# vLAR-group/OGC

Measured on AMD Instinct MI355X. Metric: point-clouds/sec (8192 pts) segnet fwd+bwd, higher is better.
Workload: dtype f32; 1 GPU; C4 KITTI-SF train_seg unsup: segnet_kitti fwd + OGC loss (dynamic+smooth+invariance) + bwd + Adam, 4 samples x 4 views x 8192 pts per GPU; n_point=8192, n_slot=10, parallelism=dp1, optimizer_stepped=True

## Files before the change

ogc_amd/csrc/neighbour_loss.hip:

```cpp
#include "ogc_common.h"

namespace {

constexpr int SUBL = 8;

__device__ __forceinline__ float sgn(float x) { return (float)((x > 0.0f) - (x < 0.0f)); }

template <int P>
__global__ __launch_bounds__(256) void nc_fwd_kernel(int n, int c, int k, const float *__restrict__ mask,
                                                     const int *__restrict__ idx, float *__restrict__ out) {
    const int b = blockIdx.y;
    const int sub = threadIdx.x & (SUBL - 1);
    const int i = blockIdx.x * (256 / SUBL) + (threadIdx.x >> 3);
    const float *mb = mask + (size_t)b * n * c;
    float acc = 0.0f;
    if (i < n) {
        const float *mi = mb + (size_t)i * c;
        const int *row = idx + ((size_t)b * n + i) * k;
        for (int j = sub; j < k; j += SUBL) {
            const float *mj = mb + (size_t)row[j] * c;
            float s = 0.0f;
            for (int ch = 0; ch < c; ++ch) {
                const float d = mi[ch] - mj[ch];
                s += P == 1 ? fabsf(d) : d * d;
            }
            acc += P == 1 ? s : sqrtf(s);
        }
    }
#pragma unroll
    for (int off = 1; off < SUBL; off <<= 1) acc += __shfl_xor(acc, off, 64);
    if (i < n && sub == 0) out[(size_t)b * n + i] = acc / (float)k;
}

constexpr unsigned REV_FIRST = 0x80000000u;

__device__ __forceinline__ bool rev_keep(const int *__restrict__ idx, long long e, int n, int k, int &dst, int &src,
                                         bool &first_dup) {
    const int j = (int)(e % k);
    src = (int)((e / k) % n);
    dst = idx[e];
    const int first = idx[e - j];
    first_dup = j > 0 && dst == first;
    return dst != src && !first_dup;
}

template <bool ROWWISE>
__global__ __launch_bounds__(256) void rev_count_kernel(long long total, int n, int k, const int *__restrict__ idx,
                                                        int *__restrict__ deg, int *__restrict__ mult) {
    const long long e = (long long)blockIdx.x * 256 + threadIdx.x;
    const bool in = e < total;
    int dst = 0, src = 0;
    bool dup = false, keep = false;
    long long b = 0;
    if (in) {
        b = e / ((long long)n * k);
        keep = rev_keep(idx, e, n, k, dst, src, dup);
    }
    if (keep) atomicAdd(&deg[b * (n + 1) + dst], 1);
    const bool extra = in && !keep && dup && dst != src;
    if (ROWWISE) {
        const unsigned long long copies = __builtin_amdgcn_ballot_w64(extra);
        const int lane = threadIdx.x & 63, row0 = lane & ~(k - 1);
        if (in && lane == row0) {
            const unsigned long long row_mask = k == 64 ? ~0ull : ((1ull << k) - 1ull) << row0;
            mult[b * n + src] = 1 + __popcll(copies & row_mask);
        }
    } else if (extra) {
        atomicAdd(&mult[b * n + src], 1);
    }
}

__global__ __launch_bounds__(1024) void rev_scan_kernel(int n, int *__restrict__ deg_to_start, int *__restrict__ cursor) {
    __shared__ int part[1024];
    const int t = threadIdx.x, b = blockIdx.x;
    int *d = deg_to_start + (size_t)b * (n + 1);
    int *cur = cursor + (size_t)b * n;
    const int per = (n + 1023) / 1024;
    const int c0 = min(t * per, n), c1 = min(c0 + per, n);
    int sum = 0;
    for (int j = c0; j < c1; ++j) sum += d[j];
    part[t] = sum;
    __syncthreads();
    for (int off = 1; off < 1024; off <<= 1) {
        const int v = t >= off ? part[t - off] : 0;
        __syncthreads();
        part[t] += v;
        __syncthreads();
    }
    int run = t > 0 ? part[t - 1] : 0;
    for (int j = c0; j < c1; ++j) {
        const int cnt = d[j];
        d[j] = run;
        cur[j] = run;
        run += cnt;
    }
    if (t == 1023) d[n] = part[1023];
}

__global__ __launch_bounds__(256) void rev_fill_kernel(long long total, int n, int k, const int *__restrict__ idx,
                                                       int *__restrict__ cursor, int *__restrict__ rev_src) {
    const long long e = (long long)blockIdx.x * 256 + threadIdx.x;
    if (e >= total) return;
    const long long b = e / ((long long)n * k);
    int dst, src;
    bool dup;
    if (!rev_keep(idx, e, n, k, dst, src, dup)) return;
    const int pos = atomicAdd(&cursor[b * n + dst], 1);
    rev_src[b * (long long)n * k + pos] = (int)((unsigned)src | (e % k == 0 ? REV_FIRST : 0u));
}

__global__ __launch_bounds__(256) void rev_sort_kernel(int n, int k, const int *__restrict__ rev_start, int *__restrict__ rev_src) {
    const int j = blockIdx.x * 256 + threadIdx.x, b = blockIdx.y;
    if (j >= n) return;
    const int *rs = rev_start + (size_t)b * (n + 1);
    int *a = rev_src + (size_t)b * n * k;
    const int lo = rs[j], hi = rs[j + 1];
    for (int i = lo + 1; i < hi; ++i) {
        const int v = a[i];
        const unsigned key = (unsigned)v & ~REV_FIRST;
        int q = i - 1;
        while (q >= lo && ((unsigned)a[q] & ~REV_FIRST) > key) {
            a[q + 1] = a[q];
            --q;
        }
        a[q + 1] = v;
    }
}

template <int P>
__device__ __forceinline__ void nc_edge(const float *a, const float *b_, int c, float w, float *g ,
                                        int stride) {
    if (P == 1) {
        for (int ch = 0; ch < c; ++ch) g[ch * stride] += w * sgn(a[ch] - b_[ch]);
    } else {
        float s = 0.0f;
        for (int ch = 0; ch < c; ++ch) { const float d = a[ch] - b_[ch]; s += d * d; }
        const float nrm = sqrtf(s);
        if (nrm > 0.0f) {
            const float inv = w / nrm;
            for (int ch = 0; ch < c; ++ch) g[ch * stride] += inv * (a[ch] - b_[ch]);
        }
    }
}

template <int P>
__global__ __launch_bounds__(256) void nc_bwd_kernel(int n, int c, int k, const float *__restrict__ mask,
                                                     const int *__restrict__ idx, const int *__restrict__ rev_start,
                                                     const int *__restrict__ rev_src,
                                                     const int *__restrict__ rev_mult,
                                                     const float *__restrict__ grad_out,
                                                     float *__restrict__ grad_mask) {
    extern __shared__ float nc_smem[];
    const int b = blockIdx.y;
    const int sub = threadIdx.x & (SUBL - 1);
    const int i = blockIdx.x * (256 / SUBL) + (threadIdx.x >> 3);
    float *g = nc_smem + threadIdx.x;
    for (int ch = 0; ch < c; ++ch) g[ch * 256] = 0.0f;
    const float *mb = mask + (size_t)b * n * c;
    const float *go = grad_out + (size_t)b * n;
    if (i < n) {
        const float *mi = mb + (size_t)i * c;
        const float inv_k = 1.0f / (float)k;
        const int *row = idx + ((size_t)b * n + i) * k;
        const float gi = go[i] * inv_k;
        for (int j = sub; j < k; j += SUBL) nc_edge<P>(mi, mb + (size_t)row[j] * c, c, gi, g, 256);
        const int *rs = rev_start + (size_t)b * (n + 1);
        const int *src = rev_src + (size_t)b * n * k;
        for (int e = rs[i] + sub; e < rs[i + 1]; e += SUBL) {
            const unsigned raw = (unsigned)src[e];
            const int ip = (int)(raw & ~REV_FIRST);
            const float times = (raw & REV_FIRST) ? (float)rev_mult[(size_t)b * n + ip] : 1.0f;
            nc_edge<P>(mb + (size_t)ip * c, mi, c, -go[ip] * inv_k * times, g, 256);
        }
    }
    __syncthreads();
    const int points = 256 / SUBL;
    for (int o = threadIdx.x; o < points * c; o += 256) {
        const int pl = o / c, ch = o % c;
        const int pi = blockIdx.x * points + pl;
        if (pi < n) {
            float s = 0.0f;
#pragma unroll
            for (int l = 0; l < SUBL; ++l) s += nc_smem[ch * 256 + pl * SUBL + l];
            grad_mask[((size_t)b * n + pi) * c + ch] = s;
        }
    }
}

}

extern "C" int ogc_neighbour_consistency_fwd(int b, int n, int c, int k, int p, const float *mask, const int *idx,
                                             float *out, ogc_stream_t stream) {
    OGC_REQUIRE(b >= 0 && n >= 0 && c >= 0 && k >= 0, "ogc_neighbour_consistency_fwd: negative size");
    OGC_REQUIRE(p == 1 || p == 2, "ogc_neighbour_consistency_fwd: norm must be 1 or 2");
    if (b == 0 || n == 0) return OGC_OK;
    OGC_REQUIRE(k > 0, "ogc_neighbour_consistency_fwd: k must be positive");
    OGC_REQUIRE(mask && idx && out, "ogc_neighbour_consistency_fwd: null pointer");
    const dim3 grid(ogc_divup(n, 256 / SUBL), b);
    if (p == 1) hipLaunchKernelGGL(nc_fwd_kernel<1>, grid, dim3(256), 0, (hipStream_t)stream, n, c, k, mask, idx, out);
    else hipLaunchKernelGGL(nc_fwd_kernel<2>, grid, dim3(256), 0, (hipStream_t)stream, n, c, k, mask, idx, out);
    OGC_CHECK_LAUNCH("ogc_neighbour_consistency_fwd");
    return OGC_OK;
}

__global__ __launch_bounds__(256) void fill_ones_kernel(long long total, int *__restrict__ p) {
    const long long e = (long long)blockIdx.x * 256 + threadIdx.x;
    if (e < total) p[e] = 1;
}

extern "C" int ogc_reverse_neighbours(int b, int n, int k, const int *idx, int *rev_start, int *rev_src, int *rev_mult,
                                      int *ws, ogc_stream_t stream) {
    OGC_REQUIRE(b >= 0 && n >= 0 && k >= 0, "ogc_reverse_neighbours: negative size");
    if (b == 0) return OGC_OK;
    OGC_REQUIRE(rev_start, "ogc_reverse_neighbours: null pointer");
    hipStream_t s = (hipStream_t)stream;
    if (ogc_zero_async(rev_start, (size_t)b * (n + 1) * sizeof(int), s) != hipSuccess) {
        ogc_set_error("ogc_reverse_neighbours: zero fill failed");
        return OGC_ERR_LAUNCH;
    }
    const long long total = (long long)b * n * k;
    if (total == 0) return OGC_OK;
    OGC_REQUIRE(idx && rev_src && rev_mult && ws, "ogc_reverse_neighbours: null pointer");
    const unsigned blocks = (unsigned)((total + 255) / 256);
    if (k <= 64 && (k & (k - 1)) == 0) {
        hipLaunchKernelGGL(rev_count_kernel<true>, dim3(blocks), dim3(256), 0, s, total, n, k, idx, rev_start, rev_mult);
    } else {
        hipLaunchKernelGGL(fill_ones_kernel, dim3(ogc_divup(b * n, 256)), dim3(256), 0, s, (long long)b * n, rev_mult);
        hipLaunchKernelGGL(rev_count_kernel<false>, dim3(blocks), dim3(256), 0, s, total, n, k, idx, rev_start,
                           rev_mult);
    }
    hipLaunchKernelGGL(rev_scan_kernel, dim3(b), dim3(1024), 0, s, n, rev_start, ws);
    hipLaunchKernelGGL(rev_fill_kernel, dim3(blocks), dim3(256), 0, s, total, n, k, idx, ws, rev_src);
    if (ogc_deterministic()) hipLaunchKernelGGL(rev_sort_kernel, dim3(ogc_divup(n, 256), b), dim3(256), 0, s, n, k, rev_start, rev_src);
    OGC_CHECK_LAUNCH("ogc_reverse_neighbours");
    return OGC_OK;
}

extern "C" int ogc_neighbour_consistency_bwd(int b, int n, int c, int k, int p, const float *mask, const int *idx,
                                             const int *rev_start, const int *rev_src, const int *rev_mult,
                                             const float *grad_out, float *grad_mask, ogc_stream_t stream) {
    OGC_REQUIRE(b >= 0 && n >= 0 && c >= 0 && k >= 0, "ogc_neighbour_consistency_bwd: negative size");
    OGC_REQUIRE(p == 1 || p == 2, "ogc_neighbour_consistency_bwd: norm must be 1 or 2");
    if (b == 0 || n == 0 || c == 0) return OGC_OK;
    OGC_REQUIRE(k > 0, "ogc_neighbour_consistency_bwd: k must be positive");
    OGC_REQUIRE(c <= 40, "ogc_neighbour_consistency_bwd: more than 40 channels");
    OGC_REQUIRE(mask && idx && rev_start && rev_src && rev_mult && grad_out && grad_mask,
                "ogc_neighbour_consistency_bwd: null pointer");
    const dim3 grid(ogc_divup(n, 256 / SUBL), b);
    const size_t smem = (size_t)c * 256 * sizeof(float);
    if (p == 1)
        hipLaunchKernelGGL(nc_bwd_kernel<1>, grid, dim3(256), smem, (hipStream_t)stream, n, c, k, mask, idx, rev_start,
                           rev_src, rev_mult, grad_out, grad_mask);
    else
        hipLaunchKernelGGL(nc_bwd_kernel<2>, grid, dim3(256), smem, (hipStream_t)stream, n, c, k, mask, idx, rev_start,
                           rev_src, rev_mult, grad_out, grad_mask);
    OGC_CHECK_LAUNCH("ogc_neighbour_consistency_bwd");
    return OGC_OK;
}
```

Baseline: 1575 point-clouds/s.

## Specialise neighbour-consistency kernels on channel width with register rows and staged indices

The forward and backward neighbour-consistency kernels are templated on channel width (4 or 10), so each point's mask row and its gradient accumulators live in registers instead of being re-read from global memory or shared memory. Each block's kNN index rows are staged into LDS, using int4 loads when alignment allows, and mask rows are read with float2 loads. Self edges are skipped, and neighbours that repeat the first neighbour (kNN padding) reuse its term through a wavefront shuffle instead of being recomputed. In exchange the code gains template variants and extra LDS use, and shared-memory accumulation is kept as a fallback for other widths.

```diff
diff --git a/ogc_amd/csrc/neighbour_loss.hip b/ogc_amd/csrc/neighbour_loss.hip
--- a/ogc_amd/csrc/neighbour_loss.hip
+++ b/ogc_amd/csrc/neighbour_loss.hip
@@ -1,4 +1,5 @@
 #include "ogc_common.h"
+#include <cstdint>
 
 namespace {
 
@@ -6,30 +7,113 @@
 
 __device__ __forceinline__ float sgn(float x) { return (float)((x > 0.0f) - (x < 0.0f)); }
 
+constexpr int NC_POINTS = 256 / SUBL;
+constexpr int NC_NARROW = 4;
+constexpr int NC_WIDE = 10;
+constexpr int NC_STAGE_K = 128;
+constexpr int NC_ROW_PAD = 8;
+
+extern __shared__ __attribute__((aligned(16))) float nc_smem[];
+
+__device__ __forceinline__ void nc_stage_rows(const int *__restrict__ src, int npts, int k, int pitch, bool vec,
+                                              int *rows) {
+    if (vec) {
+        const int total = npts * k / 4;
+        for (int q = threadIdx.x; q < total; q += 256) {
+            const int4 v = reinterpret_cast<const int4 *>(src)[q];
+            const int e = 4 * q;
+            *reinterpret_cast<int4 *>(rows + (e / k) * pitch + e % k) = v;
+        }
+    } else {
+        for (int e = threadIdx.x; e < npts * k; e += 256) rows[(e / k) * pitch + e % k] = src[e];
+    }
+}
+
+template <int CB, bool VEC>
+__device__ __forceinline__ void nc_load_row(float (&r)[CB], const float *__restrict__ p, int c) {
+    if (VEC) {
+#pragma unroll
+        for (int q = 0; q < CB / 2; ++q) {
+            float2 v = make_float2(0.0f, 0.0f);
+            if (2 * q < c) v = *reinterpret_cast<const float2 *>(p + 2 * q);
+            r[2 * q] = v.x;
+            r[2 * q + 1] = v.y;
+        }
+    } else {
+#pragma unroll
+        for (int ch = 0; ch < CB; ++ch) r[ch] = ch < c ? p[ch] : 0.0f;
+    }
+}
+
+template <int P, int CB>
+__device__ __forceinline__ float nc_norm(const float (&a)[CB], const float (&b_)[CB]) {
+    float s = 0.0f;
+#pragma unroll
+    for (int ch = 0; ch < CB; ++ch) {
+        const float d = a[ch] - b_[ch];
+        s += P == 1 ? fabsf(d) : d * d;
+    }
+    return P == 1 ? s : sqrtf(s);
+}
+
 template <int P>
+__device__ __forceinline__ float nc_norm_generic(const float *__restrict__ mi, const float *__restrict__ mj, int c) {
+    float s = 0.0f;
+    for (int ch = 0; ch < c; ++ch) {
+        const float d = mi[ch] - mj[ch];
+        s += P == 1 ? fabsf(d) : d * d;
+    }
+    return P == 1 ? s : sqrtf(s);
+}
+
+template <int P, int CB, bool VEC>
 __global__ __launch_bounds__(256) void nc_fwd_kernel(int n, int c, int k, const float *__restrict__ mask,
-                                                     const int *__restrict__ idx, float *__restrict__ out) {
+                                                     const int *__restrict__ idx, float *__restrict__ out,
+                                                     int stage, int idx_vec) {
+    int *rows = reinterpret_cast<int *>(nc_smem);
     const int b = blockIdx.y;
     const int sub = threadIdx.x & (SUBL - 1);
-    const int i = blockIdx.x * (256 / SUBL) + (threadIdx.x >> 3);
+    const int pl = threadIdx.x >> 3;
+    const int i0 = blockIdx.x * NC_POINTS;
+    const int i = i0 + pl;
+    const int pitch = k + NC_ROW_PAD;
     const float *mb = mask + (size_t)b * n * c;
-    float acc = 0.0f;
-    if (i < n) {
-        const float *mi = mb + (size_t)i * c;
-        const int *row = idx + ((size_t)b * n + i) * k;
-        for (int j = sub; j < k; j += SUBL) {
-            const float *mj = mb + (size_t)row[j] * c;
-            float s = 0.0f;
-            for (int ch = 0; ch < c; ++ch) {
-                const float d = mi[ch] - mj[ch];
-                s += P == 1 ? fabsf(d) : d * d;
+    if (stage) {
+        nc_stage_rows(idx + ((size_t)b * n + i0) * k, min(NC_POINTS, n - i0), k, pitch, idx_vec != 0, rows);
+        __syncthreads();
+    }
+    const bool live = i < n;
+    const int ic = live ? i : 0;
+    const int *grow = idx + ((size_t)b * n + ic) * k;
+    const int *lrow = rows + pl * pitch;
+    const float *mi = mb + (size_t)ic * c;
+    constexpr int CR = CB > 0 ? CB : 1;
+    float ri[CR], rj[CR];
+    if (CB > 0 && live) nc_load_row<CR, VEC>(ri, mi, c);
+    const int first = live ? (stage ? lrow[0] : grow[0]) : 0;
+    float acc = 0.0f, t_first = 0.0f;
+    for (int j0 = 0; j0 < k; j0 += SUBL) {
+        const int j = j0 + sub;
+        const bool have = live && j < k;
+        int nb = i;
+        if (have) nb = stage ? lrow[j] : grow[j];
+        const bool copy = have && j > 0 && nb == first;
+        float term = 0.0f;
+        if (have && nb != i && !copy) {
+            const float *mj = mb + (size_t)nb * c;
+            if (CB > 0) {
+                nc_load_row<CR, VEC>(rj, mj, c);
+                term = nc_norm<P, CR>(ri, rj);
+            } else {
+                term = nc_norm_generic<P>(mi, mj, c);
             }
-            acc += P == 1 ? s : sqrtf(s);
-        }
+        }
+        if (j0 == 0) t_first = __shfl(term, (threadIdx.x & 63) & ~(SUBL - 1), 64);
+        acc += copy ? t_first : term;
     }
 #pragma unroll
     for (int off = 1; off < SUBL; off <<= 1) acc += __shfl_xor(acc, off, 64);
-    if (i < n && sub == 0) out[(size_t)b * n + i] = acc / (float)k;
+    if (live && sub == 0) out[(size_t)b * n + i] = acc / (float)k;
 }
 
 constexpr unsigned REV_FIRST = 0x80000000u;
@@ -143,49 +227,133 @@
     }
 }
 
-template <int P>
+template <int P, int CB>
+__device__ __forceinline__ void nc_edge_reg(const float (&a)[CB], const float (&b_)[CB], float w, float (&v)[CB]) {
+    if (P == 1) {
+#pragma unroll
+        for (int ch = 0; ch < CB; ++ch) v[ch] = w * sgn(a[ch] - b_[ch]);
+    } else {
+        float s = 0.0f;
+#pragma unroll
+        for (int ch = 0; ch < CB; ++ch) { const float d = a[ch] - b_[ch]; s += d * d; }
+        const float nrm = sqrtf(s);
+        const float inv = w / nrm;
+#pragma unroll
+        for (int ch = 0; ch < CB; ++ch) v[ch] = nrm > 0.0f ? inv * (a[ch] - b_[ch]) : 0.0f;
+    }
+}
+
+template <int P, int CB, bool VEC>
 __global__ __launch_bounds__(256) void nc_bwd_kernel(int n, int c, int k, const float *__restrict__ mask,
                                                      const int *__restrict__ idx, const int *__restrict__ rev_start,
                                                      const int *__restrict__ rev_src,
                                                      const int *__restrict__ rev_mult,
                                                      const float *__restrict__ grad_out,
-                                                     float *__restrict__ grad_mask) {
-    extern __shared__ float nc_smem[];
+                                                     float *__restrict__ grad_mask, int stage, int idx_vec) {
     const int b = blockIdx.y;
     const int sub = threadIdx.x & (SUBL - 1);
-    const int i = blockIdx.x * (256 / SUBL) + (threadIdx.x >> 3);
+    const int pl = threadIdx.x >> 3;
+    const int i0 = blockIdx.x * NC_POINTS;
+    const int i = i0 + pl;
+    const int pitch = k + NC_ROW_PAD;
     float *g = nc_smem + threadIdx.x;
-    for (int ch = 0; ch < c; ++ch) g[ch * 256] = 0.0f;
+    float *fv = nc_smem + c * 256 + pl;
+    int *rows = reinterpret_cast<int *>(nc_smem + c * 256 + (CB > 0 ? 0 : c * NC_POINTS));
     const float *mb = mask + (size_t)b * n * c;
     const float *go = grad_out + (size_t)b * n;
-    if (i < n) {
-        const float *mi = mb + (size_t)i * c;
-        const float inv_k = 1.0f / (float)k;
-        const int *row = idx + ((size_t)b * n + i) * k;
-        const float gi = go[i] * inv_k;
-        for (int j = sub; j < k; j += SUBL) nc_edge<P>(mi, mb + (size_t)row[j] * c, c, gi, g, 256);
+    if (stage) nc_stage_rows(idx + ((size_t)b * n + i0) * k, min(NC_POINTS, n - i0), k, pitch, idx_vec != 0, rows);
+    const bool live = i < n;
+    const int ic = live ? i : 0;
+    const int *grow = idx + ((size_t)b * n + ic) * k;
+    const int *lrow = rows + pl * pitch;
+    const float *mi = mb + (size_t)ic * c;
+    const float inv_k = 1.0f / (float)k;
+    const float gi = go[ic] * inv_k;
+    constexpr int CR = CB > 0 ? CB : 1;
+    float ri[CR], rj[CR], rg[CR], rf[CR], rv[CR];
+    if (CB > 0) {
+#pragma unroll
+        for (int ch = 0; ch < CR; ++ch) rg[ch] = rf[ch] = 0.0f;
+        if (live) nc_load_row<CR, VEC>(ri, mi, c);
+    } else {
+        for (int ch = 0; ch < c; ++ch) g[ch * 256] = 0.0f;
+    }
+    if (stage) __syncthreads();
+    const int first = live ? (stage ? lrow[0] : grow[0]) : 0;
+    if (CB == 0) {
+        if (sub == 0) {
+            for (int ch = 0; ch < c; ++ch) fv[ch * NC_POINTS] = 0.0f;
+            if (live && first != i) nc_edge<P>(mi, mb + (size_t)first * c, c, gi, fv, NC_POINTS);
+        }
+        __syncthreads();
+    }
+    for (int j0 = 0; j0 < k; j0 += SUBL) {
+        const int j = j0 + sub;
+        const bool have = live && j < k;
+        int nb = i;
+        if (have) nb = stage ? lrow[j] : grow[j];
+        if (CB > 0) {
+            const bool copy = have && j > 0 && nb == first;
+#pragma unroll
+            for (int ch = 0; ch < CR; ++ch) rv[ch] = 0.0f;
+            if (have && nb != i && !copy) {
+                nc_load_row<CR, VEC>(rj, mb + (size_t)nb * c, c);
+                nc_edge_reg<P, CR>(ri, rj, gi, rv);
+            }
+            if (j0 == 0) {
+                const int lane0 = (threadIdx.x & 63) & ~(SUBL - 1);
+#pragma unroll
+                for (int ch = 0; ch < CR; ++ch) rf[ch] = __shfl(rv[ch], lane0, 64);
+            }
+#pragma unroll
+            for (int ch = 0; ch < CR; ++ch) rg[ch] += copy ? rf[ch] : rv[ch];
+        } else if (have && nb != i) {
+            if (nb == first) {
+                for (int ch = 0; ch < c; ++ch) g[ch * 256] += fv[ch * NC_POINTS];
+            } else {
+                nc_edge<P>(mi, mb + (size_t)nb * c, c, gi, g, 256);
+            }
+        }
+    }
+    if (live) {
         const int *rs = rev_start + (size_t)b * (n + 1);
         const int *src = rev_src + (size_t)b * n * k;
         for (int e = rs[i] + sub; e < rs[i + 1]; e += SUBL) {
             const unsigned raw = (unsigned)src[e];
             const int ip = (int)(raw & ~REV_FIRST);
             const float times = (raw & REV_FIRST) ? (float)rev_mult[(size_t)b * n + ip] : 1.0f;
-            nc_edge<P>(mb + (size_t)ip * c, mi, c, -go[ip] * inv_k * times, g, 256);
-        }
+            const float w = -go[ip] * inv_k * times;
+            if (CB > 0) {
+                nc_load_row<CR, VEC>(rj, mb + (size_t)ip * c, c);
+                nc_edge_reg<P, CR>(rj, ri, w, rv);
+#pragma unroll
+                for (int ch = 0; ch < CR; ++ch) rg[ch] += rv[ch];
+            } else {
+                nc_edge<P>(mb + (size_t)ip * c, mi, c, w, g, 256);
+            }
+        }
+    }
+    if (CB > 0) {
+#pragma unroll
+        for (int ch = 0; ch < CR; ++ch)
+            if (ch < c) g[ch * 256] = rg[ch];
     }
     __syncthreads();
-    const int points = 256 / SUBL;
-    for (int o = threadIdx.x; o < points * c; o += 256) {
-        const int pl = o / c, ch = o % c;
-        const int pi = blockIdx.x * points + pl;
+    for (int o = threadIdx.x; o < NC_POINTS * c; o += 256) {
+        const int ql = o / c, ch = o % c;
+        const int pi = i0 + ql;
         if (pi < n) {
             float s = 0.0f;
 #pragma unroll
-            for (int l = 0; l < SUBL; ++l) s += nc_smem[ch * 256 + pl * SUBL + l];
+            for (int l = 0; l < SUBL; ++l) s += nc_smem[ch * 256 + ql * SUBL + l];
             grad_mask[((size_t)b * n + pi) * c + ch] = s;
         }
     }
 }
+
+inline int nc_width(int c) { return c <= NC_NARROW ? NC_NARROW : c <= NC_WIDE ? NC_WIDE : 0; }
+inline bool nc_rows_vec(const float *mask, int c) { return c % 2 == 0 && reinterpret_cast<uintptr_t>(mask) % 8 == 0; }
+inline bool nc_idx_vec(const int *idx, int k) { return k % 4 == 0 && reinterpret_cast<uintptr_t>(idx) % 16 == 0; }
 
 }
 
@@ -196,9 +364,22 @@
     if (b == 0 || n == 0) return OGC_OK;
     OGC_REQUIRE(k > 0, "ogc_neighbour_consistency_fwd: k must be positive");
     OGC_REQUIRE(mask && idx && out, "ogc_neighbour_consistency_fwd: null pointer");
-    const dim3 grid(ogc_divup(n, 256 / SUBL), b);
-    if (p == 1) hipLaunchKernelGGL(nc_fwd_kernel<1>, grid, dim3(256), 0, (hipStream_t)stream, n, c, k, mask, idx, out);
-    else hipLaunchKernelGGL(nc_fwd_kernel<2>, grid, dim3(256), 0, (hipStream_t)stream, n, c, k, mask, idx, out);
+    const dim3 grid(ogc_divup(n, NC_POINTS), b);
+    const int stage = k <= NC_STAGE_K, idx_vec = nc_idx_vec(idx, k);
+    const size_t smem = stage ? (size_t)NC_POINTS * (k + NC_ROW_PAD) * sizeof(int) : 0;
+    const bool vec = nc_rows_vec(mask, c);
+#define NC_FWD(P_, CB_, VEC_)                                                                                          \
+    hipLaunchKernelGGL((nc_fwd_kernel<P_, CB_, VEC_>), grid, dim3(256), smem, (hipStream_t)stream, n, c, k, mask, idx, \
+                       out, stage, idx_vec)
+#define NC_FWD_P(P_)                                                                                                   \
+    switch (nc_width(c)) {                                                                                             \
+    case NC_NARROW: if (vec) NC_FWD(P_, NC_NARROW, true); else NC_FWD(P_, NC_NARROW, false); break;                    \
+    case NC_WIDE: if (vec) NC_FWD(P_, NC_WIDE, true); else NC_FWD(P_, NC_WIDE, false); break;                          \
+    default: NC_FWD(P_, 0, false);                                                                                     \
+    }
+    if (p == 1) { NC_FWD_P(1) } else { NC_FWD_P(2) }
+#undef NC_FWD_P
+#undef NC_FWD
     OGC_CHECK_LAUNCH("ogc_neighbour_consistency_fwd");
     return OGC_OK;
 }
@@ -246,14 +427,24 @@
     OGC_REQUIRE(c <= 40, "ogc_neighbour_consistency_bwd: more than 40 channels");
     OGC_REQUIRE(mask && idx && rev_start && rev_src && rev_mult && grad_out && grad_mask,
                 "ogc_neighbour_consistency_bwd: null pointer");
-    const dim3 grid(ogc_divup(n, 256 / SUBL), b);
-    const size_t smem = (size_t)c * 256 * sizeof(float);
-    if (p == 1)
-        hipLaunchKernelGGL(nc_bwd_kernel<1>, grid, dim3(256), smem, (hipStream_t)stream, n, c, k, mask, idx, rev_start,
-                           rev_src, rev_mult, grad_out, grad_mask);
-    else
-        hipLaunchKernelGGL(nc_bwd_kernel<2>, grid, dim3(256), smem, (hipStream_t)stream, n, c, k, mask, idx, rev_start,
-                           rev_src, rev_mult, grad_out, grad_mask);
+    const dim3 grid(ogc_divup(n, NC_POINTS), b);
+    const int width = nc_width(c);
+    const int stage = k <= NC_STAGE_K, idx_vec = nc_idx_vec(idx, k);
+    const size_t smem = ((size_t)c * 256 + (width ? 0 : (size_t)c * NC_POINTS)) * sizeof(float) +
+                        (stage ? (size_t)NC_POINTS * (k + NC_ROW_PAD) * sizeof(int) : 0);
+    const bool vec = nc_rows_vec(mask, c);
+#define NC_BWD(P_, CB_, VEC_)                                                                                          \
+    hipLaunchKernelGGL((nc_bwd_kernel<P_, CB_, VEC_>), grid, dim3(256), smem, (hipStream_t)stream, n, c, k, mask, idx, \
+                       rev_start, rev_src, rev_mult, grad_out, grad_mask, stage, idx_vec)
+#define NC_BWD_P(P_)                                                                                                   \
+    switch (width) {                                                                                                   \
+    case NC_NARROW: if (vec) NC_BWD(P_, NC_NARROW, true); else NC_BWD(P_, NC_NARROW, false); break;                    \
+    case NC_WIDE: if (vec) NC_BWD(P_, NC_WIDE, true); else NC_BWD(P_, NC_WIDE, false); break;                          \
+    default: NC_BWD(P_, 0, false);                                                                                     \
+    }
+    if (p == 1) { NC_BWD_P(1) } else { NC_BWD_P(2) }
+#undef NC_BWD_P
+#undef NC_BWD
     OGC_CHECK_LAUNCH("ogc_neighbour_consistency_bwd");
     return OGC_OK;
 }
```

New measurement: 1598 point-clouds/s (median of 5 runs). 1.5% higher.
